# Keyteer/Mixed-precision_LU_Factorization

Hardware: AMD Instinct MI355X
Metric: LU GFLOP/s at N=32768 (1/2/4/8 GPUs); IR iterations to ||r||/||b||<1e-12 (higher is better)
Workload: dtype f64

## Files before the change

### include/mpf_c.h

```cpp
#ifndef MPF_C_H
#define MPF_C_H
#include <stdint.h>
#ifdef __cplusplus
extern "C" {
#endif

typedef struct mpf_ctx mpf_ctx;

enum { MPF_TRAIL_FP64 = 0, MPF_TRAIL_FP16 = 1, MPF_TRAIL_FP16X3 = 2 };

typedef struct mpf_opts {
    int32_t trailing;
    int32_t verbose;
    int32_t fused_panel;
    int32_t sync_timing;
    int32_t no_lookahead;
    int32_t superpanel;
    int32_t pivot_path;
    int32_t reserved;
} mpf_opts;

typedef struct mpf_stats {
    double ms_total;
    double ms_h2d, ms_d2h;
// ... 27 lines not shown
int mpf_set_option(mpf_ctx *ctx, const char *name, int64_t value);
int mpf_get_option(mpf_ctx *ctx, const char *name, int64_t *value);
int mpf_option_name(int32_t index, char *buf, int64_t buflen);
int mpf_device_report(char *buf, int64_t buflen);


int mpf_factor_host(mpf_ctx *ctx, double *A_host, int64_t N, int32_t nb, int32_t *ipiv_host,
                    const mpf_opts *opts);
int mpf_trim(mpf_ctx *ctx);
int mpf_factor_dev(mpf_ctx *ctx, double *d_A, int64_t lda, int64_t N, int32_t nb, int32_t *d_ipiv,
                   const mpf_opts *opts);

int mpf_double_to_fp16(mpf_ctx *ctx, const double *d_in, uint16_t *d_out, int64_t n);
int mpf_hdiv(mpf_ctx *ctx, const uint16_t *d_a, const uint16_t *d_b, uint16_t *d_q, int64_t n);
int mpf_hgetf2_pivots(mpf_ctx *ctx, const double *d_A, int64_t lda, int32_t rows, int32_t cols,
                      int32_t ipiv_offset, int32_t *d_ipiv, uint16_t *d_panel16_out);
int mpf_hgetf2(mpf_ctx *ctx, uint16_t *d_panel16, int64_t ld, int32_t rows, int32_t cols,
               int32_t *d_ipiv_panel);
int mpf_laswp(mpf_ctx *ctx, double *d_A, int64_t lda, int64_t ncols, int32_t k, int32_t cols,
              const int32_t *d_ipiv_global);
int mpf_dgetf2_npv(mpf_ctx *ctx, double *d_P, int64_t ld, int32_t rows, int32_t cols, int32_t fused);
int mpf_dtrsm_llnu(mpf_ctx *ctx, int32_t m, int64_t n, const double *d_L, int64_t ldl, double *d_B,
                   int64_t ldb);
int mpf_dgemm_minus(mpf_ctx *ctx, int64_t m, int64_t n, int32_t k, const double *d_A, int64_t lda,
                    const double *d_B, int64_t ldb, double *d_C, int64_t ldc);

int mpf_hgemm_minus(mpf_ctx *ctx, int64_t m, int64_t n, int32_t k, const double *d_A, int64_t lda,
                    const double *d_B, int64_t ldb, double *d_C, int64_t ldc, int32_t split );

int mpf_hgemm_minus_f32(mpf_ctx *ctx, int64_t m, int64_t n, int32_t k, const double *d_A, int64_t lda,
                        const double *d_B, int64_t ldb, float *d_C, int64_t ldc, int32_t split);

int mpf_w32_from_f64(mpf_ctx *ctx, const double *d_A, int64_t lda, float *d_W, int64_t ldw, int64_t rows, int64_t cols);
int mpf_w32_to_f64(mpf_ctx *ctx, const float *d_W, int64_t ldw, double *d_A, int64_t lda, int64_t rows, int64_t cols);
int mpf_w32_laswp(mpf_ctx *ctx, float *d_W, int64_t ldw, int64_t ncols, int32_t k, int32_t cols, const int32_t *d_ipiv_global);

int mpf_matgen_dev(mpf_ctx *ctx, double *d_A, int64_t lda, int64_t N, int64_t skip);
int mpf_matgen_cols_dev(mpf_ctx *ctx, double *d_A, int64_t lda, int64_t N, int64_t skip, int64_t col0, int64_t ncols);
int mpf_matgen_state(int64_t call, uint32_t *out31);

int mpf_check_plu_dev(mpf_ctx *ctx, const double *d_A, int64_t lda, const double *d_LU, int64_t ldlu, const int32_t *d_ipiv,
                      int64_t N, double *max_abs_err, double *fro_rel_err);
int mpf_check_plu_host(const double *A, const double *LU, const int32_t *ipiv, int64_t N, double *max_abs_err, double *fro_rel_err);

typedef struct mpf_ir_stats {
    int32_t iterations;
// ... 118 lines not shown
```

### mixed-precision_lu_factorization_amd/__init__.py

```python
import ctypes as C
import os
import subprocess

_HERE = os.path.dirname(os.path.abspath(__file__))
LIB_PATH = os.environ.get("MPF_LIB") or os.path.join(_HERE, "lib", "libmpf_amd.so")
PROBE_LIB_PATH = os.environ.get("MPF_PROBE_LIB") or os.path.join(_HERE, "lib", "libmpf_probe.so")

TRAIL_FP64 = 0
TRAIL_FP16 = 1
TRAIL_FP16X3 = 2

C_ABI_SYMBOLS = [
    "mpf_create", "mpf_destroy", "mpf_set_stream", "mpf_synchronize", "mpf_last_error", "mpf_get_stats",
    "mpf_device_report", "mpf_factor_host", "mpf_factor_dev", "mpf_double_to_fp16", "mpf_hdiv",
    "mpf_hgetf2_pivots", "mpf_hgetf2", "mpf_laswp", "mpf_dgetf2_npv", "mpf_dtrsm_llnu", "mpf_dgemm_minus",
    "mpf_solve_ir", "mpf_hgetf2_capacity_rows", "mpf_set_option", "mpf_get_option", "mpf_option_name", "mpf_hgemm_minus", "mpf_hgemm_minus_f32", "mpf_w32_from_f64", "mpf_w32_to_f64", "mpf_w32_laswp", "mpf_gesv", "mpf_matgen_dev", "mpf_matgen_cols_dev",
    "mpf_matgen_state", "mpf_rccl_unique_id", "mpf_rccl_init", "mpf_rccl_destroy", "mpf_rccl_version", "mpf_rccl_info", "mpf_rccl_bcast_probe", "mpf_factor_dist",
    "mpf_solve_ir_dist", "mpf_rccl_selftest", "mpf_check_plu_dev", "mpf_check_plu_host", "mpf_solve_ir_nrhs",
    "mpf_solve_gmres_ir", "mpf_trim", "mpf_dist_set_p2p",
    "mpf_solve_ir_trans", "mpf_lange", "mpf_geequ", "mpf_gecon", "mpf_gesvx",
    "mpf_getrs", "mpf_solve_ir_block",
]
PROBE_ONLY_SYMBOLS = ["mpf_microbench", "mpf_debug_mfma4", "mpf_debug_gate", "mpf_debug_hgemm_again"]
CXX_SYMBOL_MPF = "_Z3MPFPdiiPi"


class MpfOpts(C.Structure):
    _fields_ = [("trailing", C.c_int32), ("verbose", C.c_int32), ("fused_panel", C.c_int32),
                ("sync_timing", C.c_int32), ("no_lookahead", C.c_int32), ("superpanel", C.c_int32), ("pivot_path", C.c_int32), ("reserved", C.c_int32)]


class MpfStats(C.Structure):
    _fields_ = [("ms_total", C.c_double), ("ms_h2d", C.c_double), ("ms_d2h", C.c_double),
                ("ms_hpanel", C.c_double), ("ms_laswp", C.c_double), ("ms_dpanel", C.c_double),
                ("ms_trsm", C.c_double), ("ms_gemm", C.c_double), ("n", C.c_int64), ("nb", C.c_int32),
                ("panels", C.c_int32), ("hpanel_timeouts", C.c_int32), ("info", C.c_int32),
                ("gemm_launches", C.c_int32), ("lookahead", C.c_int32), ("superpanel", C.c_int32),
                ("pivot_path", C.c_int32), ("gemm_flops", C.c_double), ("gemm_bytes", C.c_double),
                ("ms_gemm_big", C.c_double), ("gemm_big_flops", C.c_double), ("gemm_big_bytes", C.c_double),
                ("ms_cvt", C.c_double), ("ms_blockrow", C.c_double), ("gemm_big_launches", C.c_int32), ("host_rows_streamed", C.c_int32),
                ("host_late_segments", C.c_int32), ("reserved", C.c_int32)]


class MpfIrStats(C.Structure):
# ... 71 lines not shown
    L.mpf_create.argtypes = [C.POINTER(vp), C.c_int]
    L.mpf_destroy.argtypes = [vp]
    L.mpf_set_stream.argtypes = [vp, vp]
    L.mpf_synchronize.argtypes = [vp]
    L.mpf_last_error.argtypes = [vp]
    L.mpf_last_error.restype = C.c_char_p
    L.mpf_get_stats.argtypes = [vp, C.POINTER(MpfStats)]
    L.mpf_set_option.argtypes = [vp, C.c_char_p, i64]
    L.mpf_get_option.argtypes = [vp, C.c_char_p, C.POINTER(i64)]
    L.mpf_option_name.argtypes = [i32, C.c_char_p, i64]
    L.mpf_device_report.argtypes = [C.c_char_p, i64]
    L.mpf_factor_host.argtypes = [vp, vp, i64, i32, vp, C.POINTER(MpfOpts)]
    L.mpf_trim.argtypes = [vp]
    L.mpf_dist_set_p2p.argtypes = [vp, P2P_FN, vp]
    L.mpf_factor_dev.argtypes = [vp, vp, i64, i64, i32, vp, C.POINTER(MpfOpts)]
    L.mpf_double_to_fp16.argtypes = [vp, vp, vp, i64]
    L.mpf_hdiv.argtypes = [vp, vp, vp, vp, i64]
    L.mpf_hgetf2_pivots.argtypes = [vp, vp, i64, i32, i32, i32, vp, vp]
    L.mpf_hgetf2.argtypes = [vp, vp, i64, i32, i32, vp]
    L.mpf_laswp.argtypes = [vp, vp, i64, i64, i32, i32, vp]
    L.mpf_dgetf2_npv.argtypes = [vp, vp, i64, i32, i32, i32]
    L.mpf_dtrsm_llnu.argtypes = [vp, i32, i64, vp, i64, vp, i64]
    L.mpf_dgemm_minus.argtypes = [vp, i64, i64, i32, vp, i64, vp, i64, vp, i64]
    L.mpf_hgemm_minus.argtypes = [vp, i64, i64, i32, vp, i64, vp, i64, vp, i64, i32]
    L.mpf_hgemm_minus_f32.argtypes = [vp, i64, i64, i32, vp, i64, vp, i64, vp, i64, i32]
    L.mpf_w32_from_f64.argtypes = [vp, vp, i64, vp, i64, i64, i64]
    L.mpf_w32_to_f64.argtypes = [vp, vp, i64, vp, i64, i64, i64]
    L.mpf_w32_laswp.argtypes = [vp, vp, i64, i64, i32, i32, vp]
    L.mpf_solve_ir.argtypes = [vp, vp, i64, vp, i64, vp, i64, vp, vp, i32, dbl, C.POINTER(MpfIrStats)]
    L.mpf_solve_ir_nrhs.argtypes = [vp, vp, i64, vp, i64, vp, i64, i32, vp, i64, vp, i64, i32, dbl, C.POINTER(MpfIrStats)]
    L.mpf_solve_gmres_ir.argtypes = [vp, vp, i64, vp, i64, vp, i64, vp, vp, i32, i32, dbl, C.POINTER(MpfGmresStats)]
    L.mpf_gesv.argtypes = [vp, vp, i64, i64, i32, vp, vp, vp, vp, i32, dbl, i32, C.POINTER(MpfGesvStats)]
    L.mpf_solve_ir_trans.argtypes = [vp, vp, i64, vp, i64, vp, i64, i32, vp, i64, vp, i64, i32, dbl, C.POINTER(MpfIrStats)]
    L.mpf_lange.argtypes = [vp, vp, i64, i64, i64, C.c_char, C.POINTER(dbl)]
    L.mpf_geequ.argtypes = [vp, vp, i64, i64, vp, vp, C.POINTER(dbl), C.POINTER(dbl), C.POINTER(dbl)]
    L.mpf_gecon.argtypes = [vp, vp, i64, i64, C.c_char, dbl, C.POINTER(dbl), C.POINTER(MpfGeconStats)]
    L.mpf_gesvx.argtypes = [vp, vp, i64, i64, i32, vp, vp, vp, vp, i32, i32, i32, dbl, i32, dbl, vp, vp, C.POINTER(MpfGesvxStats)]
    L.mpf_getrs.argtypes = [vp, i32, vp, i64, vp, i64, i32, vp, i64]
    L.mpf_solve_ir_block.argtypes = [vp, i32, vp, i64, vp, i64, vp, i64, i32, vp, i64, vp, i64, i32, dbl, C.POINTER(MpfIrStats)]
    L.mpf_matgen_dev.argtypes = [vp, vp, i64, i64, i64]
    L.mpf_matgen_cols_dev.argtypes = [vp, vp, i64, i64, i64, i64, i64]
    L.mpf_matgen_state.argtypes = [i64, C.POINTER(C.c_uint32)]
    L.mpf_rccl_unique_id.argtypes = [vp]
    L.mpf_rccl_init.argtypes = [vp, vp, i32, i32]
    L.mpf_rccl_destroy.argtypes = [vp]
    L.mpf_rccl_version.argtypes = []
# ... 302 lines not shown
    def hgetf2(self, P16):
        self._bind()
        t = self.torch
        rows, cols = P16.shape
        ipiv = t.zeros(cols, dtype=t.int32, device=self.device)
        self._check(self.L.mpf_hgetf2(self.h, _ptr(P16), _colmajor_ld(P16), rows, cols, _ptr(ipiv)), "hgetf2")
        return ipiv

    def laswp(self, A, k, cols, ipiv_global):
        self._bind()
        self._check(self.L.mpf_laswp(self.h, _ptr(A), _colmajor_ld(A), A.shape[1], k, cols, _ptr(ipiv_global)), "laswp")

    def dgetf2_npv(self, P, fused=False):
        self._bind()
        rows, cols = P.shape
        self._check(self.L.mpf_dgetf2_npv(self.h, _ptr(P), _colmajor_ld(P), rows, cols, int(fused)), "dgetf2_npv")

    def dtrsm_llnu(self, Lm, B):
        self._bind()
        m, n = B.shape
        assert Lm.shape[0] >= m and Lm.shape[1] >= m, "dtrsm_llnu: L smaller than m x m"
        self._check(self.L.mpf_dtrsm_llnu(self.h, m, n, _ptr(Lm), _colmajor_ld(Lm), _ptr(B), _colmajor_ld(B)), "dtrsm")

    def dgemm_minus(self, Cm, A, B):
        self._bind()
        m, n = Cm.shape
        k = A.shape[1]
        assert A.shape == (m, k) and B.shape == (k, n), "dgemm_minus: operand shapes do not match C"
        self._check(self.L.mpf_dgemm_minus(self.h, m, n, k, _ptr(A), _colmajor_ld(A), _ptr(B), _colmajor_ld(B),
                                           _ptr(Cm), _colmajor_ld(Cm)), "dgemm")

    def hgemm_minus(self, Cm, A, B, split=False):
        self._bind()
        m, n = Cm.shape
        k = A.shape[1]
        assert A.shape == (m, k) and B.shape == (k, n), "hgemm_minus: operand shapes do not match C"
        self._check(self.L.mpf_hgemm_minus(self.h, m, n, k, _ptr(A), _colmajor_ld(A), _ptr(B), _colmajor_ld(B),
                                           _ptr(Cm), _colmajor_ld(Cm), int(split)), "hgemm")

    def hgemm_minus_f32(self, Cm, A, B, split=False):
        self._bind()
        assert Cm.dtype == self.torch.float32
        m, n = Cm.shape
        k = A.shape[1]
        assert A.shape == (m, k) and B.shape == (k, n), "hgemm_minus_f32: operand shapes do not match C"
        self._check(self.L.mpf_hgemm_minus_f32(self.h, m, n, k, _ptr(A), _colmajor_ld(A), _ptr(B), _colmajor_ld(B),
# ... 130 lines not shown
```

### mixed-precision_lu_factorization_amd/csrc/mpf_host.cpp

```cpp
#include "mpf_internal.h"
#include "../../include/MPF.h"
#include <climits>
#include <cstdio>
#include <cstdlib>
#include <cstring>
#include <cmath>
#include <iostream>
#include <vector>
#include <mutex>
#include <functional>
#include <chrono>

static thread_local std::string g_noctx_err;

namespace {
struct OptDesc { const char *name, *env; size_t off; bool wide; long long lo, hi; };
#define OPT_I(field, env, lo, hi) {#field, env, offsetof(MpfTuning, field), false, lo, hi}
#define OPT_L(field, env, lo, hi) {#field, env, offsetof(MpfTuning, field), true, lo, hi}
const OptDesc kOpts[] = {
    OPT_I(safe_pivots, "MPF_SAFE_PIVOTS", 0, 1),
    OPT_I(chain_pipeline, "MPF_CHAIN_PIPELINE", 0, 1),
    OPT_L(chain_pipeline_below, "MPF_CHAIN_PIPELINE_BELOW", 0, 1ll << 40),
    OPT_I(fp16_work32, "MPF_FP16_WORK32", 0, 1),
    OPT_I(superpanel_fp16, "MPF_SUPERPANEL", 0, 8),
// ... 3 lines not shown
    OPT_I(timeline, "MPF_TIMELINE", 0, 1),
    OPT_L(hp_spin_limit, "MPF_HP_SPIN_LIMIT", 1, 1ll << 31),
    OPT_L(hp_gate_ticks, "MPF_HP_GATE_TICKS", 0, 1ll << 40),
    OPT_I(hp_acq_fence, "MPF_HP_ACQ_FENCE", 0, 1),
    OPT_I(hp_window, "MPF_HP_WINDOW", -1, 1 << 30),
    OPT_I(hgemm_pad, "MPF_HGEMM_PAD", 0, 65536),
    OPT_I(hgemm_split_pad, "MPF_HGEMM_SPLIT_PAD", 0, 65536),
    OPT_I(hgemm_big, "MPF_HGEMM_BIG", 0, 1),
    OPT_I(hgemm_big_tile, "MPF_HGEMM_BIG_TILE", 0, 5),
    OPT_I(hgemm_mfma16, "MPF_HGEMM_MFMA16", 0, 1),
    OPT_I(dgemm_dma, "MPF_DGEMM_DMA", 0, 1),
    OPT_I(lazy_gather, "MPF_LAZY_GATHER", 0, 1),
    OPT_I(dpanel_fused_form, "MPF_DPANEL_FUSED", 0, 1),
    OPT_I(dist_instalments, "MPF_DIST_INSTALMENTS", 0, 1),
    OPT_L(dist_instalment_min_bytes, "MPF_DIST_INSTALMENT_MIN_BYTES", 0, 1ll << 40),
    OPT_I(generic_fused, "MPF_GENERIC_FUSED", 0, 1),
    OPT_I(fp64_rowmajor, "MPF_FP64_ROWMAJOR", 0, 1),
    OPT_L(fp64_rowmajor_min_n, "MPF_FP64_ROWMAJOR_MIN_N", 0, 1ll << 40),
    OPT_I(trsm_laswp_fused, "MPF_TRSM_LASWP_FUSED", 0, 1),
    OPT_I(fp64_two_lanes, "MPF_FP64_TWO_LANES", 0, 1 << 30),
    OPT_I(fp64_lane_a_pct, "MPF_FP64_LANE_A_PCT", 20, 90),
    OPT_I(fp64_pair, "MPF_FP64_PAIR", 0, 1),
    OPT_L(fp64_pair_min_n, "MPF_FP64_PAIR_MIN_N", 0, 1ll << 40),
    OPT_I(event_timers, "MPF_EVENT_TIMERS", 0, 2),
    OPT_I(dist_world1_loop, "MPF_DIST_WORLD1_LOOP", 0, 1),
    OPT_I(gesv_fp64_tflops, "MPF_GESV_FP64_TFLOPS", 0, 1000),
    OPT_I(gate_wait_value, "MPF_GATE_WAIT_VALUE", 0, 1),
    OPT_I(host_sink, "MPF_HOST_SINK", 0, 1),
    OPT_I(sink_trace, "MPF_SINK_TRACE", 0, 1),
    OPT_I(hp_half_slabs, "MPF_HP_HALF_SLABS", 0, 1),
    OPT_I(hp_half_slabs_rows, "MPF_HP_HALF_SLABS_ROWS", 256, 32768),
    OPT_I(hp_local_xcd, "MPF_HP_LOCAL_XCD", 0, 2),
    OPT_I(host_late_parts, "MPF_HOST_LATE_PARTS", 0, 4),
    OPT_L(host_late_min_n, "MPF_HOST_LATE_MIN_N", 0, 1ll << 40),
    OPT_I(host_first_pct, "MPF_HOST_FIRST_PCT", 5, 100),
    OPT_I(host_late_q_pct, "MPF_HOST_LATE_Q_PCT", 1, 1000),
    OPT_L(host_sink_min_n, "MPF_HOST_SINK_MIN_N", 0, 1ll << 40),
    OPT_I(dist_solve_p2p, "MPF_DIST_SOLVE_P2P", 0, 1),
#ifdef MPF_PROBE
    OPT_I(hp_stamp, "MPF_HP_STAMP", 0, 1),
    OPT_I(hp_r256_upto, "MPF_HP_R256_UPTO", 0, 1 << 30),
    OPT_I(dgemm_w8, "MPF_DGEMM_W8", 0, 1),
    OPT_I(gemm_lds_pad, "MPF_GEMM_LDS_PAD", 0, 65536),
    OPT_I(hgemm_big_reg, "MPF_HGEMM_BIG_REG", 0, 1),
    OPT_I(hgemm_dbg, "MPF_HGEMM_DBG", 0, 8191),
#endif
// ... 186 lines not shown
    return launch_hgetf2_generic(c, d_A, lda, nullptr, 0, rows, cols, ipiv_offset, d_ipiv, d_panel16_out, rows);
}
int mpf_hgetf2(mpf_ctx *c, uint16_t *d_panel16, int64_t ld, int32_t rows, int32_t cols, int32_t *d_ipiv_panel) {
    if (!c || !d_panel16 || !d_ipiv_panel) return -1;
    if (ld < rows) return fail(c, -1, "hgetf2: ld < rows");
    if (!safe_pivots(c) && hgetf2_lds_eligible(c, rows, cols))
        return launch_hgetf2(c, nullptr, 0, d_panel16, ld, rows, cols, 0, d_ipiv_panel, nullptr, 0, nullptr);
    return launch_hgetf2_generic(c, nullptr, 0, d_panel16, ld, rows, cols, 0, d_ipiv_panel, nullptr, 0);
}
int mpf_laswp(mpf_ctx *c, double *d_A, int64_t lda, int64_t ncols, int32_t k, int32_t cols, const int32_t *d_ipiv) {
    if (!c || !d_A || !d_ipiv) return -1;
    if (cols > HP_MAXCOLS) return launch_laswp_seq(c, d_A, lda, ncols, k, cols, d_ipiv, lda);
    return launch_laswp(c, d_A, lda, ncols, k, cols, d_ipiv);
}
int mpf_dgetf2_npv(mpf_ctx *c, double *d_P, int64_t ld, int32_t rows, int32_t cols, int32_t fused) {
    if (!c || !d_P) return -1;
    if (ld < rows) return fail(c, -1, "dgetf2_npv: ld < rows");
    return launch_dgetf2_npv(c, d_P, ld, rows, cols, fused, 0);
}
int mpf_dtrsm_llnu(mpf_ctx *c, int32_t m, int64_t n, const double *d_L, int64_t ldl, double *d_B, int64_t ldb) {
    if (!c) return -1;
    if (m > 0 && n > 0 && (ldl < m || ldb < m)) return fail(c, -1, "dtrsm: leading dimension < m");
    return launch_dtrsm_llnu(c, m, n, d_L, ldl, d_B, ldb);
}
int mpf_dgemm_minus(mpf_ctx *c, int64_t m, int64_t n, int32_t k, const double *d_A, int64_t lda, const double *d_B,
                    int64_t ldb, double *d_C, int64_t ldc) {
    if (!c) return -1;
    if (m > 0 && n > 0 && k > 0 && (lda < m || ldb < k || ldc < m)) return fail(c, -1, "dgemm: bad leading dimension");
    return launch_dgemm_minus(c, m, n, k, d_A, lda, d_B, ldb, d_C, ldc);
}

int mpf_ensure_h_images(mpf_ctx *c, int64_t rows, int kmax, bool big) {
    kmax = (kmax + 63) & ~63;
    if (c->h_L && c->h_rows >= rows && c->h_kmax >= kmax && (!big || c->h_Lb[0])) return 0;
    if (rows < c->h_rows) rows = c->h_rows;
    if (kmax < c->h_kmax) kmax = c->h_kmax;
    big = big || c->h_Lb[0];
    c->h_L.release(); c->h_U.release();
    for (auto &b : c->h_Lb) b.release();
    c->h_rows = 0; c->h_kmax = 0;
    const int64_t elems = 2 * rows * kmax;
    MPF_HIP_TRY(c, c->h_L.grow(elems));
    MPF_HIP_TRY(c, c->h_U.grow(elems));
    if (big) for (auto &b : c->h_Lb) MPF_HIP_TRY(c, b.grow(elems));
    c->h_rows = rows; c->h_kmax = kmax;
    return 0;
// ... 417 lines not shown
            if (!rc) rc = ev.timed(st.ms_trsm, T, [&] { return launch_dtrsm_llnu_strided(c, nb, nb, Ak1, lda, R + k1 * ldr + k2, ldr, 1); });
            hipStreamWaitEvent(T, pi_ready, 0);
            if (!rc) rc = ev.timed(st.ms_gemm, T, [&] { return launch_dgemm_minus(c, nb, N - k2, nb, R + k1 * ldr + k2, ldr, PI2 + nb, ldp, R + k2 * ldr + k2, ldr); });
            count_gemm(st, o, N - k2, nb, nb);
            if (!rc) rc = ev.timed(st.ms_cvt, T, [&] { return launch_transpose64(c, d_A + k2 * lda + k2, lda, R + k2 * ldr + k2, ldr, N - k2, nb, false); });
            hipEventRecord(e2, T);
            if (!rc) rc = ev.timed(st.ms_cvt, T, [&] { return launch_transpose64(c, d_A + k2 * lda + k1, lda, R + k1 * ldr + k2, ldr, nb, nb, false); });
        }
        if (rc) break;
        {
            hipStreamWaitEvent(P, e2, 0);
            if (doneB) hipStreamWaitEvent(P, doneB, 0);
            hipEventRecord(ps2, P);
            rc = panel_chain(f, k2, P);
            hipEventRecord(chain2, P);
        }
        if (rc) break;
        auto far_prep = [&](int64_t c_lo, int64_t w) -> int {
            const int64_t off = (int64_t)LASWP_MAXMOVED * c_lo;
            int e = ev.timed(st.ms_laswp, T, [&] {
                int e2_ = launch_laswp_from_list_rm64(c, R + c_lo, ldr, w, lk, off);
                if (!e2_) e2_ = launch_laswp_from_list_rm64(c, R + c_lo, ldr, w, lk1, off);
                return e2_; });
            if (!e) e = ev.timed(st.ms_trsm, T, [&] { return launch_dtrsm_llnu_strided(c, nb, w, Ak, lda, R + k * ldr + c_lo, ldr, 1); });
            if (!e) e = ev.timed(st.ms_gemm, T, [&] { return launch_dgemm_minus(c, w, nb, nb, R + k * ldr + c_lo, ldr, PI, ldp, R + k1 * ldr + c_lo, ldr); });
            count_gemm(st, o, nb, w, nb);
            if (!e) e = ev.timed(st.ms_trsm, T, [&] { return launch_dtrsm_llnu_strided(c, nb, w, Ak1, lda, R + k1 * ldr + c_lo, ldr, 1); });
            if (!e) e = ev.timed(st.ms_cvt, T, [&] { return launch_transpose64(c, d_A + c_lo * lda + k, lda, R + k * ldr + c_lo, ldr, 2 * nb, w, false); });
            return e;
        };
        {
            if (doneA) hipStreamWaitEvent(T, doneA, 0); else hipStreamWaitEvent(T, init_done, 0);
            if (resplit && doneB) hipStreamWaitEvent(T, doneB, 0);
            StreamSwap sw(c, T);
            rc = far_prep(k3, k5 - k3);
            hipEventRecord(evX, T);
            if (!rc) rc = far_prep(k5, cm - k5);
            hipEventRecord(evA, T);
        }
        if (rc) break;
        hipStreamWaitEvent(S, evX, 0);
        hipStreamWaitEvent(S, ps2, 0);
        rc = far_update(k, PI2, k3, k5 - k3);
        if (rc) break;
        doneX = ev.get();
        hipEventRecord(doneX, S);
        hipStreamWaitEvent(S, evA, 0);
        rc = far_update(k, PI2, k5, cm - k5);
        if (rc) break;
        doneA = ev.get();
// ... 797 lines not shown
```

### mixed-precision_lu_factorization_amd/csrc/mpf_internal.h

```cpp
#pragma once
#include <hip/hip_runtime.h>
#include <stdint.h>
#include <string>
#include <vector>
#include <functional>
#include "../../include/mpf_c.h"

constexpr int HP_R = 256;
constexpr int HP_T = 512;
constexpr int HP_MAXG = 256;
constexpr int HP_MAXCOLS = 256;
constexpr int LASWP_MAXMOVED = 2 * HP_MAXCOLS;

struct MovedList {
    int n;
    int pad[3];
    int src[LASWP_MAXMOVED];
    int dst[LASWP_MAXMOVED];
};

struct MpfWorkspace {
    unsigned long long cand[2][HP_MAXG];
    int flags[16];
    unsigned long long rowbuf[2][HP_MAXG][HP_MAXCOLS / 2];
// ... 35 lines not shown
    int generic_fused = 1;
    int fp64_rowmajor = 1;
    long long fp64_rowmajor_min_n = 8192;
    int trsm_laswp_fused = 1;
    int fp64_two_lanes = 8192;
    int dist_solve_p2p = 0;
    int host_sink = 1;
    int hp_local_xcd = 1;
    int hp_half_slabs = 1;
    int hp_half_slabs_rows = 16384;
    int sink_trace = 0;
    int host_late_parts = 3;
    long long host_late_min_n = 16384;
    int host_first_pct = 25;
    int host_late_q_pct = 110;
    long long host_sink_min_n = 4096;
    int gate_wait_value = 0;
    int gesv_fp64_tflops = 0;
    int dist_world1_loop = 0;
    int event_timers = 1;
    int fp64_lane_a_pct = 50;
    int fp64_pair = 1;
    long long fp64_pair_min_n = 16384;
#ifdef MPF_PROBE
    int hp_stamp = 0;
    int hp_r256_upto = 1 << 30;
    int dgemm_w8 = 1;
    int gemm_lds_pad = 0;
    int hgemm_dbg = 0;
    int hgemm_big_reg = 0;
#endif
};

template <class T, bool Pinned = false>
struct Buf {
    Buf() = default;
    Buf(const Buf &) = delete;
    Buf &operator=(const Buf &) = delete;
    ~Buf() { release(); }
    hipError_t grow(int64_t n) {
        if (n <= cap_) return hipSuccess;
        release();
        void *q = nullptr;
        const hipError_t e = Pinned ? hipHostMalloc(&q, (size_t)n * sizeof(T)) : hipMalloc(&q, (size_t)n * sizeof(T));
        if (e != hipSuccess) return e;
        p_ = (T *)q;
// ... 71 lines not shown
    Buf<unsigned short> g16;
    Buf<unsigned long long> gcand;
    void *rccl_comm = nullptr;
    int rccl_rank = 0, rccl_world = 0;
    long long rccl_bcast_calls = 0, rccl_bcast_bytes = 0, rccl_allreduce_calls = 0, rccl_p2p_calls = 0, rccl_p2p_bytes = 0;
    Buf<double> dist_buf[2];
    Buf<float> dist_w32;
    Buf<double> dist_spl;
    int hp_resident_per_cu = -1;
    int hp_win_per_cu = 0;
    int hp_full_beside_waiter = 0;
    int hp_win_beside_waiter = 0;
};

#define MPF_HIP_TRY(ctx, expr)                                                        \
    do {                                                                              \
        hipError_t e_ = (expr);                                                       \
        if (e_ != hipSuccess) {                                                       \
            (ctx)->err = std::string(#expr) + ": " + hipGetErrorString(e_);           \
            return -2;                                                                \
        }                                                                             \
    } while (0)

enum { ATTR_HP = 1, ATTR_DGEMM = 2, ATTR_HGEMM = 4, ATTR_HGEMM256 = 8, ATTR_HGEMM_PP = 16, ATTR_HGEMM16_BIG32 = 32, ATTR_HGEMM16_BIG64 = 64 };
inline bool safe_pivots(const mpf_ctx *c) { return c->tune.safe_pivots != 0; }

int launch_double_to_fp16(mpf_ctx *c, const double *in, uint16_t *out, int64_t n);
int launch_hdiv(mpf_ctx *c, const uint16_t *a, const uint16_t *b, uint16_t *q, int64_t n);
int launch_hgetf2(mpf_ctx *c, const double *A64, int64_t lda, uint16_t *P16, int64_t ld16, int rows,
                  int cols, int ipiv_offset, int *d_ipiv, uint16_t *out16, int64_t ldo, MovedList *moved, int waiters = 0, int prefer_window_rows = 0);
bool hgetf2_lds_eligible(mpf_ctx *c, int rows, int cols);
bool hgetf2_fits_beside(mpf_ctx *c, int rows, int cols, int waiters);
long long hgetf2_capacity_rows(mpf_ctx *c, int waiters, int form = 0);
int laswp_gated_footprint(int *lds_bytes, int *vgprs, int *threads);
int laswp_gated_grid(int64_t ncols);
constexpr int HP_FP64_WINDOW_ROWS = 20000;
int hp_query_residency(mpf_ctx *c);
int launch_hgetf2_gate(mpf_ctx *c, int target);
int launch_laswp_block(mpf_ctx *c, double *A, int64_t lda, int64_t ncols, int k, int cols, const int *d_ipiv, int64_t nrows);
int launch_laswp_block_gated(mpf_ctx *c, double *A, int64_t lda, int64_t ncols, int k, int cols, const int *d_ipiv, int64_t nrows, int target);
int dgetf2_npv_pieces(mpf_ctx *c, int cols);
int launch_dgetf2_npv_piece(mpf_ctx *c, double *P, int64_t ld, int rows, int cols, int fused, int info_base, int piece);
int launch_dpanel_tile_copy(mpf_ctx *c, double *dst, int64_t ld, int piece);
int launch_hgetf2_generic(mpf_ctx *c, const double *A64, int64_t lda, uint16_t *P16, int64_t ld16, int rows, int cols,
                          int ipiv_offset, int *d_ipiv, uint16_t *out16, int64_t ldo);
int launch_laswp_seq(mpf_ctx *c, double *A, int64_t lda, int64_t ncols, int k, int cols, const int *d_ipiv, int64_t nrows);
int launch_laswp_from_list(mpf_ctx *c, double *A, int64_t lda, int64_t ncols, const MovedList *ml);
// ... 27 lines not shown
int launch_dgetf2_npv(mpf_ctx *c, double *P, int64_t ld, int rows, int cols, int fused, int info_base);
int launch_dtrsm_llnu(mpf_ctx *c, int m, int64_t n, const double *L, int64_t ldl, double *B, int64_t ldb);
int launch_dgemm_minus(mpf_ctx *c, int64_t m, int64_t n, int k, const double *A, int64_t lda,
                       const double *B, int64_t ldb, double *C, int64_t ldc);
int launch_cvt_l21(mpf_ctx *c, const double *A, int64_t lda, int64_t m, int K, int split, int img = 0, int64_t elem_off = 0);
int launch_hgemm_minus(mpf_ctx *c, int64_t m, int64_t n, int K, const double *B, int64_t ldb, double *C, int64_t ldc,
                       int split, int img = 0, int64_t elem_off = 0);
int launch_hgemm_minus_w32(mpf_ctx *c, int64_t m, int64_t n, int K, const double *B, int64_t ldb, float *C, int64_t ldc,
                           int split, int img = 0, int64_t elem_off = 0);
int launch_cvt_u12(mpf_ctx *c, const double *B, int64_t ldb, int K, int64_t n, int split, int64_t elem_off = 0, int kstride = 0);
int launch_hgemm_images(mpf_ctx *c, int64_t m, int64_t n, int K, void *C, int64_t ldc, bool c32, int split, int img = 0, int64_t elem_off = 0,
                        int64_t u_off = 0, int ksL = 0, int ksU = 0);
struct HgemmImages { const unsigned short *Lh = nullptr, *Ll = nullptr, *Uh = nullptr, *Ul = nullptr; int ksL = 0, ksU = 0; };
int launch_hgemm_ptrs(mpf_ctx *c, int64_t m, int64_t n, int K, const HgemmImages &im, void *C, int64_t ldc, bool c32, int split);
int launch_hgemm16_big(mpf_ctx *c, int64_t m, int64_t n, int Kp, const HgemmImages &im, void *C, int64_t ldc, bool c32);
int launch_hgemm16_ring(mpf_ctx *c, int64_t m, int64_t n, int Kp, const HgemmImages &im, void *C, int64_t ldc, bool c32);
int launch_hgemm_pp(mpf_ctx *c, int64_t m, int64_t n, int Kp, const HgemmImages &im, float *C, int64_t ldc);
int launch_hgemm_images_rowmajor(mpf_ctx *c, int64_t m, int64_t n, int K, float *Crm, int64_t ldrow, int split, int img = 0, int64_t elem_off = 0,
                                 int64_t u_off = 0, int ksL = 0, int ksU = 0);
int launch_laswp_from_list_f32(mpf_ctx *c, float *A, int64_t lda, int64_t ncols, const MovedList *ml);
int launch_laswp_from_list_rm64(mpf_ctx *c, double *R, int64_t ldr, int64_t ncols, const MovedList *ml, int64_t scratch_off = 0);
int launch_transpose64(mpf_ctx *c, double *A, int64_t lda, double *R, int64_t ldr, int64_t rows, int64_t cols, bool to_rowmajor);
int launch_dtrsm_llnu_strided(mpf_ctx *c, int m, int64_t n, const double *L, int64_t ldl, double *B, int64_t rs, int64_t cs);
int launch_cvt_f64_f32(mpf_ctx *c, const double *A, int64_t lda, float *W, int64_t ldw, int64_t rows, int64_t cols);
int launch_cvt_f32_f64(mpf_ctx *c, const float *W, int64_t ldw, double *A, int64_t lda, int64_t rows, int64_t cols);
int launch_gather_rows(mpf_ctx *c, const double *in, const int *perm, double *out, int64_t n);
int launch_residual(mpf_ctx *c, const double *A, int64_t lda, const double *x, const double *b, double *r,
                    int64_t n);
int launch_residual_rect(mpf_ctx *c, const double *A, int64_t lda, const double *x, const double *b, double *r, int64_t n, int64_t ncols);
int launch_trsv_prepare_cols(mpf_ctx *c, const double *LUb, int64_t ld, int64_t n, int64_t k0, int w);
int launch_trsv_lower_cols(mpf_ctx *c, const double *LUb, int64_t ld, double *x, int64_t n, int64_t k0, int w);
int launch_trsv_upper_cols(mpf_ctx *c, const double *LUb, int64_t ld, double *x, int64_t n, int64_t k0, int w);
extern "C" {
int mpf_ensure_h_images(mpf_ctx *c, int64_t rows, int kmax, bool big);
int mpf_ensure_solve_buf(mpf_ctx *c, int64_t n);
int mpf_ensure_rowmajor_copy(mpf_ctx *c, int64_t rows, int64_t cols, int32_t nb);
int mpf_factor_setup(mpf_ctx *c, int64_t N, int32_t nb, int32_t npanels, bool lists);
}
int launch_trsv_prepare(mpf_ctx *c, const double *LU, int64_t ld, int64_t n);
int launch_trsv_lower_unit(mpf_ctx *c, const double *LU, int64_t ld, double *x, int64_t n);
int launch_trsv_upper(mpf_ctx *c, const double *LU, int64_t ld, double *x, int64_t n);
int launch_axpy(mpf_ctx *c, double alpha, const double *x, double *y, int64_t n);
int launch_norm2(mpf_ctx *c, const double *x, int64_t n, double *d_out);
int launch_dot(mpf_ctx *c, const double *x, const double *y, int64_t n, double *d_out);
int launch_scal(mpf_ctx *c, double alpha, double *x, int64_t n);
int solve_setup(mpf_ctx *c, const double *d_LU, int64_t ldlu, const int32_t *d_ipiv, int64_t N);
// ... 77 lines not shown
```

### mixed-precision_lu_factorization_amd/csrc/trailing_f64.hip

```cpp
#include "mpf_internal.h"

typedef double d4_t __attribute__((ext_vector_type(4)));
typedef double d2_t __attribute__((ext_vector_type(2)));
typedef unsigned u2_t __attribute__((ext_vector_type(2)));

__device__ __forceinline__ double buf_load_f64(__amdgpu_buffer_rsrc_t rsrc, unsigned voff, unsigned soff) {
    const u2_t v = __builtin_amdgcn_raw_buffer_load_b64(rsrc, (int)voff, (int)soff, 0);
    return __builtin_bit_cast(double, v);
}
__device__ __forceinline__ __amdgpu_buffer_rsrc_t make_rsrc(const void *p) {
    return __builtin_amdgcn_make_buffer_rsrc(const_cast<void *>(p), 0, 0x7FFFFFFF, 0x00020000);
}

constexpr int GT = 128;
constexpr int GBK = 16;
constexpr int GSA = 144;
constexpr int GSB = GBK + 2;
constexpr int G_LDS_DOUBLES = 2 * GBK * GSA + 2 * GT * GSB;
#ifndef DMA_NEG_BLGP
#define DMA_NEG_BLGP 2
#endif


template <bool EDGE, int NT>
// ... 435 lines not shown
                                R[t][g] = __builtin_amdgcn_mfma_f64_16x16x4f64(lf[t][kk], xg[g][kk], R[t][g], 0, 0, 1 );
                    }
                }
                if (bj + 2 < mt) load_l(bj + 1, lf);
            }
        }
    }
#pragma unroll
    for (int t = 0; t < 4; ++t)
#pragma unroll
        for (int g = 0; g < CG; ++g)
#pragma unroll
            for (int r = 0; r < 4; ++r) {
                const int row = (w + 4 * t) * TR_T + lk + 4 * r;
                if (cok[g] && row < m) B[row * rs + coff[g]] = R[t][g][r];
            }
}

static void dtrsm_launch(mpf_ctx *c, int m, int64_t n, const double *L, int64_t ldl, double *B, int64_t rs, int64_t cs) {
    if (n <= 12288) dtrsm_llnu_kernel<1><<<(int)((n + 15) / 16), 256, 0, c->stream>>>(m, n, L, ldl, B, rs, cs);
    else dtrsm_llnu_kernel<4><<<(int)((n + 63) / 64), 256, 0, c->stream>>>(m, n, L, ldl, B, rs, cs);
}

int launch_dtrsm_llnu(mpf_ctx *c, int m, int64_t n, const double *L, int64_t ldl, double *B, int64_t ldb) {
    if (m <= 0 || n <= 0) return 0;
    for (int i0 = 0; i0 < m; i0 += TR_T * TR_MAXT) {
        const int mb = (m - i0) < TR_T * TR_MAXT ? (m - i0) : TR_T * TR_MAXT;
        if (i0 > 0) {
            const int rc = launch_dgemm_minus(c, mb, n, i0, L + i0, ldl, B, ldb, B + i0, ldb);
            if (rc) return rc;
        }
        dtrsm_launch(c, mb, n, L + i0 + (long long)i0 * ldl, ldl, B + i0, 1, ldb);
    }
    MPF_HIP_TRY(c, hipGetLastError());
    return 0;
}
int launch_dtrsm_llnu_strided(mpf_ctx *c, int m, int64_t n, const double *L, int64_t ldl, double *B, int64_t rs, int64_t cs) {
    if (m <= 0 || n <= 0) return 0;
    if (m > TR_T * TR_MAXT) { c->err = "dtrsm (strided): at most 256 rows"; return -1; }
    dtrsm_launch(c, m, n, L, ldl, B, rs, cs);
    MPF_HIP_TRY(c, hipGetLastError());
    return 0;
}
```

Baseline: 54490.

## Fuse paired-panel TRSM, GEMM and TRSM into one stacked block-triangular solve kernel

Adds a stacked lower-unit-triangular solve kernel that treats two consecutive panels (L1, L2 and the off-diagonal coupling block P) as one 2nb-row block-triangular system. In the FP64 pair path it replaces a sequence of three launches (trsm, gemm update, trsm) with one kernel, enabled by default through a new option. The kernel pre-inverts the diagonal 16x16 blocks in LDS and sweeps block columns with f64 MFMA, passing solved blocks between waves through LDS. This removes launch overhead and intermediate global round trips, at the cost of register pressure, more complex code, and stride limits on the factor operands.

```diff
diff --git a/include/mpf_c.h b/include/mpf_c.h
--- a/include/mpf_c.h
+++ b/include/mpf_c.h
@@ -73,6 +73,10 @@
 int mpf_dgetf2_npv(mpf_ctx *ctx, double *d_P, int64_t ld, int32_t rows, int32_t cols, int32_t fused);
 int mpf_dtrsm_llnu(mpf_ctx *ctx, int32_t m, int64_t n, const double *d_L, int64_t ldl, double *d_B,
                    int64_t ldb);
+int mpf_dtrsm_llnu_strided(mpf_ctx *ctx, int32_t m, int64_t n, const double *d_L, int64_t ldl, double *d_B,
+                           int64_t rs, int64_t cs);
+int mpf_dtrsm_llnu_stacked(mpf_ctx *ctx, int32_t m1, int32_t m2, int64_t n, const double *d_L1, const double *d_L2,
+                           int64_t ldl, const double *d_P, int64_t pr, int64_t pc, double *d_B, int64_t rs, int64_t cs);
 int mpf_dgemm_minus(mpf_ctx *ctx, int64_t m, int64_t n, int32_t k, const double *d_A, int64_t lda,
                     const double *d_B, int64_t ldb, double *d_C, int64_t ldc);
 
diff --git a/mixed-precision_lu_factorization_amd/__init__.py b/mixed-precision_lu_factorization_amd/__init__.py
--- a/mixed-precision_lu_factorization_amd/__init__.py
+++ b/mixed-precision_lu_factorization_amd/__init__.py
@@ -20,6 +20,7 @@
     "mpf_solve_gmres_ir", "mpf_trim", "mpf_dist_set_p2p",
     "mpf_solve_ir_trans", "mpf_lange", "mpf_geequ", "mpf_gecon", "mpf_gesvx",
     "mpf_getrs", "mpf_solve_ir_block",
+    "mpf_dtrsm_llnu_strided", "mpf_dtrsm_llnu_stacked",
 ]
 PROBE_ONLY_SYMBOLS = ["mpf_microbench", "mpf_debug_mfma4", "mpf_debug_gate", "mpf_debug_hgemm_again"]
 CXX_SYMBOL_MPF = "_Z3MPFPdiiPi"
@@ -137,6 +138,8 @@
     L.mpf_dgetf2_npv.argtypes = [vp, vp, i64, i32, i32, i32]
     L.mpf_dtrsm_llnu.argtypes = [vp, i32, i64, vp, i64, vp, i64]
     L.mpf_dgemm_minus.argtypes = [vp, i64, i64, i32, vp, i64, vp, i64, vp, i64]
+    L.mpf_dtrsm_llnu_strided.argtypes = [vp, i32, i64, vp, i64, vp, i64, i64]
+    L.mpf_dtrsm_llnu_stacked.argtypes = [vp, i32, i32, i64, vp, vp, i64, vp, i64, i64, vp, i64, i64]
     L.mpf_hgemm_minus.argtypes = [vp, i64, i64, i32, vp, i64, vp, i64, vp, i64, i32]
     L.mpf_hgemm_minus_f32.argtypes = [vp, i64, i64, i32, vp, i64, vp, i64, vp, i64, i32]
     L.mpf_w32_from_f64.argtypes = [vp, vp, i64, vp, i64, i64, i64]
@@ -485,6 +488,21 @@
         assert Lm.shape[0] >= m and Lm.shape[1] >= m, "dtrsm_llnu: L smaller than m x m"
         self._check(self.L.mpf_dtrsm_llnu(self.h, m, n, _ptr(Lm), _colmajor_ld(Lm), _ptr(B), _colmajor_ld(B)), "dtrsm")
 
+    def dtrsm_llnu_strided(self, Lm, B):
+        self._bind()
+        m, n = B.shape
+        assert Lm.shape[0] >= m and Lm.shape[1] >= m, "dtrsm_llnu_strided: L smaller than m x m"
+        self._check(self.L.mpf_dtrsm_llnu_strided(self.h, m, n, _ptr(Lm), _colmajor_ld(Lm), _ptr(B), B.stride(0), B.stride(1)), "dtrsm")
+
+    def dtrsm_llnu_stacked(self, L1, L2, P, B):
+        self._bind()
+        m1, m2 = L1.shape[0], L2.shape[0]
+        assert L1.shape[1] >= m1 and L2.shape[1] >= m2 and P.shape == (m2, m1) and B.shape[0] == m1 + m2, "dtrsm_llnu_stacked: shapes"
+        ld = _colmajor_ld(L1)
+        assert _colmajor_ld(L2) == ld, "dtrsm_llnu_stacked: L1 and L2 need one leading dimension"
+        self._check(self.L.mpf_dtrsm_llnu_stacked(self.h, m1, m2, B.shape[1], _ptr(L1), _ptr(L2), ld, _ptr(P), P.stride(0), P.stride(1),
+                                                  _ptr(B), B.stride(0), B.stride(1)), "dtrsm_stacked")
+
     def dgemm_minus(self, Cm, A, B):
         self._bind()
         m, n = Cm.shape
diff --git a/mixed-precision_lu_factorization_amd/csrc/mpf_host.cpp b/mixed-precision_lu_factorization_amd/csrc/mpf_host.cpp
--- a/mixed-precision_lu_factorization_amd/csrc/mpf_host.cpp
+++ b/mixed-precision_lu_factorization_amd/csrc/mpf_host.cpp
@@ -49,6 +49,7 @@
     OPT_I(fp64_lane_a_pct, "MPF_FP64_LANE_A_PCT", 20, 90),
     OPT_I(fp64_pair, "MPF_FP64_PAIR", 0, 1),
     OPT_L(fp64_pair_min_n, "MPF_FP64_PAIR_MIN_N", 0, 1ll << 40),
+    OPT_I(fp64_stack, "MPF_FP64_STACK", 0, 1),
     OPT_I(event_timers, "MPF_EVENT_TIMERS", 0, 2),
     OPT_I(dist_world1_loop, "MPF_DIST_WORLD1_LOOP", 0, 1),
     OPT_I(gesv_fp64_tflops, "MPF_GESV_FP64_TFLOPS", 0, 1000),
@@ -281,6 +282,17 @@
     if (!c) return -1;
     if (m > 0 && n > 0 && (ldl < m || ldb < m)) return fail(c, -1, "dtrsm: leading dimension < m");
     return launch_dtrsm_llnu(c, m, n, d_L, ldl, d_B, ldb);
+}
+int mpf_dtrsm_llnu_strided(mpf_ctx *c, int32_t m, int64_t n, const double *d_L, int64_t ldl, double *d_B, int64_t rs, int64_t cs) {
+    if (!c) return -1;
+    if (m > 0 && n > 0 && ldl < m) return fail(c, -1, "dtrsm: leading dimension < m");
+    return launch_dtrsm_llnu_strided(c, m, n, d_L, ldl, d_B, rs, cs);
+}
+int mpf_dtrsm_llnu_stacked(mpf_ctx *c, int32_t m1, int32_t m2, int64_t n, const double *d_L1, const double *d_L2, int64_t ldl,
+                           const double *d_P, int64_t pr, int64_t pc, double *d_B, int64_t rs, int64_t cs) {
+    if (!c) return -1;
+    if (n > 0 && (ldl < m1 || ldl < m2)) return fail(c, -1, "dtrsm (stacked): leading dimension < m");
+    return launch_dtrsm_llnu_stacked(c, m1, m2, n, d_L1, d_L2, ldl, d_P, pr, pc, d_B, rs, cs);
 }
 int mpf_dgemm_minus(mpf_ctx *c, int64_t m, int64_t n, int32_t k, const double *d_A, int64_t lda, const double *d_B,
                     int64_t ldb, double *d_C, int64_t ldc) {
@@ -744,10 +756,15 @@
                 int e2_ = launch_laswp_from_list_rm64(c, R + c_lo, ldr, w, lk, off);
                 if (!e2_) e2_ = launch_laswp_from_list_rm64(c, R + c_lo, ldr, w, lk1, off);
                 return e2_; });
-            if (!e) e = ev.timed(st.ms_trsm, T, [&] { return launch_dtrsm_llnu_strided(c, nb, w, Ak, lda, R + k * ldr + c_lo, ldr, 1); });
-            if (!e) e = ev.timed(st.ms_gemm, T, [&] { return launch_dgemm_minus(c, w, nb, nb, R + k * ldr + c_lo, ldr, PI, ldp, R + k1 * ldr + c_lo, ldr); });
-            count_gemm(st, o, nb, w, nb);
-            if (!e) e = ev.timed(st.ms_trsm, T, [&] { return launch_dtrsm_llnu_strided(c, nb, w, Ak1, lda, R + k1 * ldr + c_lo, ldr, 1); });
+            if (c->tune.fp64_stack) {
+                if (!e) e = ev.timed(st.ms_trsm, T, [&] { return launch_dtrsm_llnu_stacked(c, nb, nb, w, Ak, Ak1, lda, PI, ldp, 1, R + k * ldr + c_lo, ldr, 1); });
+                st.gemm_flops += 2.0 * (double)nb * (double)w * (double)nb;
+            } else {
+                if (!e) e = ev.timed(st.ms_trsm, T, [&] { return launch_dtrsm_llnu_strided(c, nb, w, Ak, lda, R + k * ldr + c_lo, ldr, 1); });
+                if (!e) e = ev.timed(st.ms_gemm, T, [&] { return launch_dgemm_minus(c, w, nb, nb, R + k * ldr + c_lo, ldr, PI, ldp, R + k1 * ldr + c_lo, ldr); });
+                count_gemm(st, o, nb, w, nb);
+                if (!e) e = ev.timed(st.ms_trsm, T, [&] { return launch_dtrsm_llnu_strided(c, nb, w, Ak1, lda, R + k1 * ldr + c_lo, ldr, 1); });
+            }
             if (!e) e = ev.timed(st.ms_cvt, T, [&] { return launch_transpose64(c, d_A + c_lo * lda + k, lda, R + k * ldr + c_lo, ldr, 2 * nb, w, false); });
             return e;
         };
diff --git a/mixed-precision_lu_factorization_amd/csrc/mpf_internal.h b/mixed-precision_lu_factorization_amd/csrc/mpf_internal.h
--- a/mixed-precision_lu_factorization_amd/csrc/mpf_internal.h
+++ b/mixed-precision_lu_factorization_amd/csrc/mpf_internal.h
@@ -81,6 +81,7 @@
     int fp64_lane_a_pct = 50;
     int fp64_pair = 1;
     long long fp64_pair_min_n = 16384;
+    int fp64_stack = 1;
 #ifdef MPF_PROBE
     int hp_stamp = 0;
     int hp_r256_upto = 1 << 30;
@@ -198,7 +199,7 @@
         }                                                                             \
     } while (0)
 
-enum { ATTR_HP = 1, ATTR_DGEMM = 2, ATTR_HGEMM = 4, ATTR_HGEMM256 = 8, ATTR_HGEMM_PP = 16, ATTR_HGEMM16_BIG32 = 32, ATTR_HGEMM16_BIG64 = 64 };
+enum { ATTR_HP = 1, ATTR_DGEMM = 2, ATTR_HGEMM = 4, ATTR_HGEMM256 = 8, ATTR_HGEMM_PP = 16, ATTR_HGEMM16_BIG32 = 32, ATTR_HGEMM16_BIG64 = 64, ATTR_DTRSM_STACK = 128 };
 inline bool safe_pivots(const mpf_ctx *c) { return c->tune.safe_pivots != 0; }
 
 int launch_double_to_fp16(mpf_ctx *c, const double *in, uint16_t *out, int64_t n);
@@ -272,6 +273,8 @@
 int launch_laswp_from_list_rm64(mpf_ctx *c, double *R, int64_t ldr, int64_t ncols, const MovedList *ml, int64_t scratch_off = 0);
 int launch_transpose64(mpf_ctx *c, double *A, int64_t lda, double *R, int64_t ldr, int64_t rows, int64_t cols, bool to_rowmajor);
 int launch_dtrsm_llnu_strided(mpf_ctx *c, int m, int64_t n, const double *L, int64_t ldl, double *B, int64_t rs, int64_t cs);
+int launch_dtrsm_llnu_stacked(mpf_ctx *c, int m1, int m2, int64_t n, const double *L1, const double *L2, int64_t ldl, const double *P,
+                              int64_t pr, int64_t pc, double *B, int64_t rs, int64_t cs);
 int launch_cvt_f64_f32(mpf_ctx *c, const double *A, int64_t lda, float *W, int64_t ldw, int64_t rows, int64_t cols);
 int launch_cvt_f32_f64(mpf_ctx *c, const float *W, int64_t ldw, double *A, int64_t lda, int64_t rows, int64_t cols);
 int launch_gather_rows(mpf_ctx *c, const double *in, const int *perm, double *out, int64_t n);
diff --git a/mixed-precision_lu_factorization_amd/csrc/trailing_f64.hip b/mixed-precision_lu_factorization_amd/csrc/trailing_f64.hip
--- a/mixed-precision_lu_factorization_amd/csrc/trailing_f64.hip
+++ b/mixed-precision_lu_factorization_amd/csrc/trailing_f64.hip
@@ -1,4 +1,5 @@
 #include "mpf_internal.h"
+#include <utility>
 
 typedef double d4_t __attribute__((ext_vector_type(4)));
 typedef double d2_t __attribute__((ext_vector_type(2)));
@@ -481,6 +482,205 @@
     else dtrsm_llnu_kernel<4><<<(int)((n + 63) / 64), 256, 0, c->stream>>>(m, n, L, ldl, B, rs, cs);
 }
 
+constexpr int TS_MAXT = 32;
+constexpr int TS_TW = TS_MAXT / 4;
+template <int... I, class F> __device__ __forceinline__ void static_for_ts(std::integer_sequence<int, I...>, F &&f) {
+    (f(std::integral_constant<int, I>{}), ...);
+}
+template <int CG> constexpr int ts_lds_bytes() { return (4 * TS_TW * 256 + 2 * CG * 64 * 4) * 8; }
+
+__device__ __forceinline__ int ts_brow(int bi, int r, bool &ok, int t1, int m1, int m2) {
+    const bool lo = bi >= t1;
+    const int loc = (lo ? bi - t1 : bi) * TR_T + r;
+    ok = loc < (lo ? m2 : m1);
+    return ok ? (lo ? m1 + loc : loc) : 0;
+}
+__device__ __forceinline__ void ts_load_l(int bj, double (&f)[TS_TW][4], int w, int li, int lk, int t1, int m1, int m2, const double *__restrict__ L1,
+                                          const double *__restrict__ L2, long long ldl, const double *__restrict__ P, long long pr, long long pc) {
+    const bool jlo = bj >= t1;
+    const int jb = (jlo ? bj - t1 : bj) * TR_T + lk, klim = jlo ? m2 : m1;
+#pragma unroll
+    for (int t = 0; t < TS_TW; ++t) {
+        if (4 * t + 3 <= bj) continue;
+        const int bi = w + 4 * t;
+        if (bi > bj) {
+            const bool ilo = bi >= t1, off = ilo && !jlo;
+            const int gi = (ilo ? bi - t1 : bi) * TR_T + li;
+            const bool iok = gi < (ilo ? m2 : m1);
+            const char *base = (const char *)(ilo ? (jlo ? L2 : P) : L1);
+            const unsigned sr = (unsigned)(off ? pr : 1), sc = (unsigned)(off ? pc : ldl);
+            const unsigned ro = (unsigned)(iok ? gi : 0) * sr;
+            double v[4];
+#pragma unroll
+            for (int kk = 0; kk < 4; ++kk) {
+                const int gk = jb + 4 * kk;
+                v[kk] = *(const double *)(base + (size_t)((ro + (unsigned)(gk < klim ? gk : 0) * sc) * 8u));
+            }
+            asm volatile("" : "+v"(v[0]), "+v"(v[1]), "+v"(v[2]), "+v"(v[3]));
+#pragma unroll
+            for (int kk = 0; kk < 4; ++kk) f[t][kk] = (iok && jb + 4 * kk < klim) ? v[kk] : 0.0;
+        }
+    }
+}
+
+template <int CG>
+__global__ __launch_bounds__(256, 2) void dtrsm_llnu_stacked_kernel(int m1, int m2, long long n, const double *__restrict__ L1,
+                                                                    const double *__restrict__ L2, long long ldl,
+                                                                    const double *__restrict__ P, long long pr, long long pc,
+                                                                    double *B, long long rs, long long cs) {
+    extern __shared__ __attribute__((aligned(16))) double sh_stack[];
+    double *sh = sh_stack;
+    const int tid = threadIdx.x, lane = tid & 63, w = __builtin_amdgcn_readfirstlane(tid >> 6);
+    const int t1 = (m1 + TR_T - 1) / TR_T, mt = t1 + (m2 + TR_T - 1) / TR_T;
+    const int li = lane & 15, lk = lane >> 4;
+    auto brow = [&](int bi, int r, bool &ok) __attribute__((always_inline)) -> int { return ts_brow(bi, r, ok, t1, m1, m2); };
+
+    long long coff[CG];
+    bool cok[CG];
+#pragma unroll
+    for (int g = 0; g < CG; ++g) {
+        const long long col = ((long long)blockIdx.x * CG + g) * 16 + li;
+        cok[g] = col < n;
+        coff[g] = (cok[g] ? col : 0) * cs;
+    }
+    d4_t R[TS_TW][CG];
+#pragma unroll
+    for (int g = 0; g < CG; ++g)
+#pragma unroll
+        for (int h = 0; h < 2; ++h) {
+            double v[16];
+#pragma unroll
+            for (int q = 0; q < 16; ++q) {
+                bool ok;
+                const int row = brow(w + 4 * (4 * h + (q >> 2)), lk + 4 * (q & 3), ok);
+                v[q] = B[row * rs + coff[g]];
+            }
+            KEEP16(v);
+#pragma unroll
+            for (int q = 0; q < 16; ++q) {
+                bool ok;
+                brow(w + 4 * (4 * h + (q >> 2)), lk + 4 * (q & 3), ok);
+                R[4 * h + (q >> 2)][g][q & 3] = ok ? v[q] : 0.0;
+            }
+        }
+    auto load_l = [&](int bj, double (&f)[TS_TW][4]) __attribute__((always_inline)) { ts_load_l(bj, f, w, li, lk, t1, m1, m2, L1, L2, ldl, P, pr, pc); };
+    double lf[TS_TW][4];
+    if (mt > 1) load_l(0, lf);
+    double *shw = sh + w * (TS_TW * 256);
+#pragma unroll 1
+    for (int h = 0; h < 2; ++h) {
+        double *shh = shw + h * 1024;
+        {
+            double v[16];
+            bool keep[16];
+#pragma unroll
+            for (int q = 0; q < 16; ++q) {
+                const int e = lane + 64 * q, tt = e >> 8, j = (e >> 4) & 15, i = e & 15;
+                const int bi = w + 4 * (4 * h + tt);
+                const bool lo = bi >= t1;
+                const int gi = (lo ? bi - t1 : bi) * TR_T + i, gj = (lo ? bi - t1 : bi) * TR_T + j, lim = lo ? m2 : m1;
+                keep[q] = i > j && gi < lim && gj < lim;
+                v[q] = (lo ? L2 : L1)[(gi < lim ? gi : 0) + (long long)(gj < lim ? gj : 0) * ldl];
+            }
+            KEEP16(v);
+#pragma unroll
+            for (int q = 0; q < 16; ++q) shh[lane + 64 * q] = keep[q] ? v[q] : 0.0;
+        }
+        __syncthreads();
+        {
+            const int tt = lane >> 4, c = lane & 15;
+            const double *lt = shh + tt * 256;
+            double x[TR_T];
+#pragma unroll
+            for (int i = 0; i < TR_T; ++i) x[i] = (i == c) ? 1.0 : 0.0;
+#pragma unroll
+            for (int j = 0; j < TR_T; ++j)
+#pragma unroll
+                for (int i = j + 1; i < TR_T; ++i) {
+                    x[i] = __builtin_fma(-lt[j * 16 + i], x[j], x[i]);
+                    if (i == TR_T - 1) __builtin_amdgcn_sched_barrier(0);
+                }
+            __syncthreads();
+#pragma unroll
+            for (int i = 0; i < TR_T; ++i) shh[tt * 256 + c * 16 + i] = x[i];
+        }
+    }
+    __syncthreads();
+    d4_t *slot = reinterpret_cast<d4_t *>(sh + 4 * TS_TW * 256);
+
+    static_for_ts(std::make_integer_sequence<int, TS_MAXT>{}, [&](auto bjc) __attribute__((always_inline)) {
+        constexpr int bj = decltype(bjc)::value;
+        if (bj < mt) {
+            constexpr int to = bj >> 2;
+            const bool owner = (w == (bj & 3));
+            d4_t xg[CG];
+            if (owner) {
+                double inv[4];
+#pragma unroll
+                for (int kk = 0; kk < 4; ++kk) inv[kk] = shw[to * 256 + (4 * kk + lk) * 16 + li];
+#pragma unroll
+                for (int g = 0; g < CG; ++g) {
+                    d4_t acc = (d4_t){0.0, 0.0, 0.0, 0.0};
+#pragma unroll
+                    for (int kk = 0; kk < 4; ++kk) acc = __builtin_amdgcn_mfma_f64_16x16x4f64(inv[kk], R[to][g][kk], acc, 0, 0, 0);
+                    xg[g] = acc;
+                    R[to][g] = acc;
+                }
+                if (bj + 1 < mt) {
+#pragma unroll
+                    for (int g = 0; g < CG; ++g) slot[((bj & 1) * CG + g) * 64 + lane] = xg[g];
+                }
+            }
+            if (bj + 1 < mt) {
+                asm volatile("s_waitcnt lgkmcnt(0)" ::: "memory");
+                __builtin_amdgcn_s_barrier();
+                asm volatile("" ::: "memory");
+                if (!owner) {
+#pragma unroll
+                    for (int g = 0; g < CG; ++g) xg[g] = slot[((bj & 1) * CG + g) * 64 + lane];
+                }
+#pragma unroll
+                for (int t = 0; t < TS_TW; ++t) {
+                    if (4 * t + 3 > bj && w + 4 * t > bj) {
+#pragma unroll
+                        for (int g = 0; g < CG; ++g)
+#pragma unroll
+                            for (int kk = 0; kk < 4; ++kk)
+                                R[t][g] = __builtin_amdgcn_mfma_f64_16x16x4f64(lf[t][kk], xg[g][kk], R[t][g], 0, 0, 1 );
+                    }
+                }
+                if (bj + 2 < mt) load_l(bj + 1, lf);
+            }
+        }
+    });
+#pragma unroll
+    for (int t = 0; t < TS_TW; ++t)
+#pragma unroll
+        for (int g = 0; g < CG; ++g)
+#pragma unroll
+            for (int r = 0; r < 4; ++r) {
+                bool ok;
+                const int row = brow(w + 4 * t, lk + 4 * r, ok);
+                if (cok[g] && ok) B[row * rs + coff[g]] = R[t][g][r];
+            }
+}
+
+int launch_dtrsm_llnu_stacked(mpf_ctx *c, int m1, int m2, int64_t n, const double *L1, const double *L2, int64_t ldl, const double *P,
+                              int64_t pr, int64_t pc, double *B, int64_t rs, int64_t cs) {
+    if (m1 < 0 || m2 < 0 || m1 > TR_T * TR_MAXT || m2 > TR_T * TR_MAXT) { c->err = "dtrsm (stacked): at most 256 rows per block"; return -1; }
+    if (n <= 0 || m1 + m2 == 0) return 0;
+    if (m2 == 0) return launch_dtrsm_llnu_strided(c, m1, n, L1, ldl, B, rs, cs);
+    if (m1 == 0) return launch_dtrsm_llnu_strided(c, m2, n, L2, ldl, B, rs, cs);
+    if (!(c->attr_done & ATTR_DTRSM_STACK)) {
+        MPF_HIP_TRY(c, hipFuncSetAttribute((const void *)dtrsm_llnu_stacked_kernel<1>, hipFuncAttributeMaxDynamicSharedMemorySize, ts_lds_bytes<1>()));
+        c->attr_done |= ATTR_DTRSM_STACK;
+    }
+    if (ldl > (1ll << 20) || pr < 0 || pc < 0 || pr > (1ll << 20) || pc > (1ll << 20)) { c->err = "dtrsm (stacked): stride of a factor operand above 2^20"; return -1; }
+    dtrsm_llnu_stacked_kernel<1><<<(int)((n + 15) / 16), 256, ts_lds_bytes<1>(), c->stream>>>(m1, m2, n, L1, L2, ldl, P, pr, pc, B, rs, cs);
+    MPF_HIP_TRY(c, hipGetLastError());
+    return 0;
+}
+
 int launch_dtrsm_llnu(mpf_ctx *c, int m, int64_t n, const double *L, int64_t ldl, double *B, int64_t ldb) {
     if (m <= 0 || n <= 0) return 0;
     for (int i0 = 0; i0 < m; i0 += TR_T * TR_MAXT) {
```

Result: slower. 53930 (-1.0%).
